# jopohl/urh

Measured on NVIDIA H100. Metric: MSamples/s IQ demod+digitize (complex64), higher is better.
Workload: dtype f32

## Files before the change

### urh_b200/csrc/dense_f32.cuh

```cuda
#pragma once
#include "dense.cuh"

struct SrcQad {
    static constexpr bool BINARY = false;
    template <typename T> __device__ __forceinline__ static int cls(T s, const UrhClassify& C, float) { return urh_classify((float)s, C); }
    template <typename T> __device__ __forceinline__ static void bits(T, const UrhClassify&, float, bool& nz, bool& ab) { nz = false; ab = false; }
    template <typename T> __device__ __forceinline__ static bool above(T, float) { return false; }
};
struct SrcQad2 {
    static constexpr bool BINARY = true;
    template <typename T> __device__ __forceinline__ static int cls(T s, const UrhClassify& C, float thr0) {
        const int c = ((float)s <= thr0) ? 0 : 1;
        return ((float)s == C.noise_value) ? -1 : c;
    }
    template <typename T> __device__ __forceinline__ static void bits(T s, const UrhClassify& C, float thr0, bool& nz, bool& ab) {
        nz = (float)s == C.noise_value;
        ab = !((float)s <= thr0) && !nz;
    }
    template <typename T> __device__ __forceinline__ static bool above(T s, float thr0) { return !((float)s <= thr0); }
};
struct SrcAbove {
    static constexpr bool BINARY = true;
    template <typename T> __device__ __forceinline__ static int cls(T s, const UrhClassify&, float thr0) { return (s > (T)thr0) ? 1 : 0; }
    template <typename T> __device__ __forceinline__ static void bits(T s, const UrhClassify&, float thr0, bool& nz, bool& ab) { nz = false; ab = s > (T)thr0; }
    template <typename T> __device__ __forceinline__ static bool above(T s, float thr0) { return s > (T)thr0; }
};
struct SrcCenter {
    static constexpr bool BINARY = true;
    template <typename T> __device__ __forceinline__ static int cls(T s, const UrhClassify&, float thr0) { return (s <= (T)thr0) ? 0 : 1; }
    template <typename T> __device__ __forceinline__ static void bits(T s, const UrhClassify&, float thr0, bool& nz, bool& ab) { nz = false; ab = !(s <= (T)thr0); }
    template <typename T> __device__ __forceinline__ static bool above(T s, float thr0) { return !(s <= (T)thr0); }
};

struct UrhSpec {
    const float* tg;
    float* margin;
    int64_t lo, hi;
    unsigned int* redone;
};

template <typename T> struct UrhVec2;
template <> struct UrhVec2<float> { typedef float2 type; };
template <> struct UrhVec2<double> { typedef double2 type; };

template <typename SRC, typename T>
__global__ void __launch_bounds__(URH_WARPS_PER_BLOCK * 32)
k_dense_f32(const T* __restrict__ x, int64_t n, int vec_in, const __grid_constant__ UrhClassify cls, int tol,
            UrhTileSummary* __restrict__ tiles, uint32_t* __restrict__ staging, int stage_cap,
            int16_t* __restrict__ init_cls, int cls_of_zero, const float* __restrict__ d_thr0 = nullptr,
            const UrhTileStats* __restrict__ tile_stats = nullptr, const UrhSpec spec = UrhSpec{}) {
    const float thr0 = d_thr0 ? *d_thr0 : cls.thr[0];
    if (d_thr0) cls_of_zero = (0.0f <= thr0) ? 0 : 1;
    const int lane = threadIdx.x & 31;
    const int64_t tile = (int64_t)blockIdx.x * URH_WARPS_PER_BLOCK + (threadIdx.x >> 5);
    const int64_t tile_start = tile * URH_TILE;
    if (tile_start >= n) return;
    const int tile_len = (int)((n - tile_start) < URH_TILE ? (n - tile_start) : URH_TILE);
    const int iters = (tile_len + 63) >> 6;
    if (tile_stats && tile_stats[tile].all_noise) {
        if (lane == 0) {
            UrhTileSummary s;
            s.first_cls = -1; s.last_cls = -1; s.head_len = tile_len; s.tail_len = tile_len; s.ncand = 0;
            tiles[tile] = s;
            if (tile_start == 0 && init_cls) *init_cls = (int16_t)-1;
        }
        return;
    }
    if (tile >= spec.lo && tile < spec.hi) {
        if (spec.margin[tile] > fabsf(__fsub_rn(thr0, *spec.tg))) return;
        if (lane == 0) atomicAdd(spec.redone, 1u);
    }
    UrhRunTracker rt;
    rt.init(tol, staging + tile * (int64_t)stage_cap);
    if (vec_in && tile_len == URH_TILE) {
        typedef typename UrhVec2<T>::type V;
        const V* p = (const V*)(x + tile_start) + lane;
        constexpr int ITERS = URH_TILE / 64;
        const bool no_noise = SRC::BINARY && tile_stats && cls.noise_value <= -4.0f && tile_stats[tile].cnt == URH_TILE;
        V cur[4], nxt[4];
#pragma unroll
        for (int j = 0; j < 4; j++) cur[j] = __ldg(p + j * 32);
        if (tile_start == 0 && lane == 0 && init_cls) *init_cls = (int16_t)(((float)cur[0].x == cls.noise_value) ? -1 : cls_of_zero);
        if (SRC::BINARY) {
            UrhTileResolve tr;
            tr.init();
#pragma unroll 1
            for (int it = 0; it < ITERS; it += 4) {
                if (it + 4 < ITERS) {
#pragma unroll
                    for (int j = 0; j < 4; j++) nxt[j] = __ldg(p + (it + 4 + j) * 32);
                }
                if (no_noise) {
#pragma unroll
                    for (int j = 0; j < 4; j++)
                        tr.keep(it + j, 0u, __ballot_sync(URH_FULL_MASK, SRC::template above<T>(cur[j].x, thr0)), 0u,
                                __ballot_sync(URH_FULL_MASK, SRC::template above<T>(cur[j].y, thr0)), lane);
                } else {
#pragma unroll
                    for (int j = 0; j < 4; j++) {
                        bool nx, ax, ny, ay;
                        SRC::template bits<T>(cur[j].x, cls, thr0, nx, ax);
                        SRC::template bits<T>(cur[j].y, cls, thr0, ny, ay);
                        tr.keep(it + j, __ballot_sync(URH_FULL_MASK, nx), __ballot_sync(URH_FULL_MASK, ax), __ballot_sync(URH_FULL_MASK, ny),
                                __ballot_sync(URH_FULL_MASK, ay), lane);
// ... 17 lines not shown
#pragma unroll
            for (int j = 0; j < 4; j++) cur[j] = nxt[j];
        }
        rt.finish(tile_len, tiles + tile, lane);
        return;
    }
    for (int it = 0; it < iters; it += 2) {
        T a0 = 0, a1 = 0, b0 = 0, b1 = 0;
        const int64_t pa = tile_start + (int64_t)it * 64 + 2 * lane;
        const int64_t pb = pa + 64;
        if (vec_in && pa + 1 < n) {
            const typename UrhVec2<T>::type v = __ldg((const typename UrhVec2<T>::type*)(x + pa));
            a0 = v.x; a1 = v.y;
        } else {
            if (pa < n) a0 = __ldg(x + pa);
            if (pa + 1 < n) a1 = __ldg(x + pa + 1);
        }
        const bool has_b = it + 1 < iters;
        if (has_b) {
            if (vec_in && pb + 1 < n) {
                const typename UrhVec2<T>::type v = __ldg((const typename UrhVec2<T>::type*)(x + pb));
                b0 = v.x; b1 = v.y;
            } else {
                if (pb < n) b0 = __ldg(x + pb);
                if (pb + 1 < n) b1 = __ldg(x + pb + 1);
            }
        }
        if (pa == 0 && init_cls) *init_cls = (int16_t)(((float)a0 == cls.noise_value) ? -1 : cls_of_zero);
        rt.feed(it, SRC::template cls<T>(a0, cls, thr0), SRC::template cls<T>(a1, cls, thr0), pa < n, pa + 1 < n, lane);
        if (has_b) rt.feed(it + 1, SRC::template cls<T>(b0, cls, thr0), SRC::template cls<T>(b1, cls, thr0), pb < n, pb + 1 < n, lane);
    }
    rt.finish(tile_len, tiles + tile, lane);
}
```

### urh_b200/csrc/digitize.cu

```cuda
#include "dense.cuh"
#include "scan.cuh"
#include "sparse.cuh"
#ifndef URH_FAST_MIN_BLOCKS
#define URH_FAST_MIN_BLOCKS 4
#endif
#include "fsk_fast.cuh"
#include "dense_f32.cuh"

#include <math.h>
#include <stdlib.h>


template <int DT, int MOD, bool DIGITIZE>
__device__ __forceinline__ void dense_iq_tile(const void* __restrict__ iq, int64_t n, const UrhDemodParams& dp, float* __restrict__ qad_out,
                                              int vec_in, int vec_out, const UrhClassify& cls, int tol, UrhTileSummary* __restrict__ tiles,
                                              uint32_t* __restrict__ staging, int stage_cap, int16_t* __restrict__ init_cls, int cls_of_zero,
                                              int64_t tile, int has_halo, UrhTileStats* __restrict__ tile_stats, const UrhFine& fine,
                                              unsigned int* s_fine, unsigned int* g_fine) {
    const int lane = threadIdx.x & 31;
    const int64_t tile_start = tile * URH_TILE;
    const int tile_len = (int)((n - tile_start) < URH_TILE ? (n - tile_start) : URH_TILE);
    const int iters = (tile_len + 63) >> 6;

    UrhRunTracker rt;
// ... 805 lines not shown
    if (urh_iq_bytes(dtype) == 0) URH_FAIL(ctx, URH_ERR_DTYPE, "Unsupported dtype");
    return URH_OK;
}

static int stream_check(urh_ctx* ctx, int64_t n, int ring, int mod_type, int dtype, bool iq) {
    if (n <= 0) URH_FAIL(ctx, URH_ERR_INVALID, "streamed call: empty capture");
    if (ring < 2 || ring > URH_STREAM_MAX_RING) URH_FAIL(ctx, URH_ERR_INVALID, "streamed call: ring of %d slots (2..%d)", ring, URH_STREAM_MAX_RING);
    if (iq && (n <= 2 || (mod_type != URH_MOD_ASK && mod_type != URH_MOD_FSK)))
        URH_FAIL(ctx, URH_ERR_INVALID, "streamed demodulation: ASK/FSK and n > 2 (PSK is a serial recurrence)");
    if (iq && urh_iq_bytes(dtype) == 0) URH_FAIL(ctx, URH_ERR_DTYPE, "Unsupported dtype");
    return URH_OK;
}

template <bool DIG>
static int stream_dense_iq(urh_ctx* ctx, int dtype, int mod_type, const char* d_src, int64_t src_slot, int64_t n, const UrhDemodParams& dp,
                           float* qad_global, const UrhClassify& cls, int tol, StreamDigitizer* dz, int64_t s0, int64_t s1, int s,
                           UrhTileStats* ts = nullptr, const UrhFine& fine = UrhFine{}) {
    const int b = urh_iq_bytes(dtype);
    const void* iq = d_src + s * src_slot + URH_STREAM_PAD - s0 * b;
    const int64_t t0 = s0 / URH_TILE, t1 = urh_div_up(s1, URH_TILE);
    UrhTileSummary* tiles = dz ? dz->tiles - t0 : nullptr;
    uint32_t* staging = dz ? dz->staging - t0 * dz->cap : nullptr;
    const int cap = dz ? dz->cap : 0;
    int16_t* init = dz ? dz->d_init : nullptr;
    const int c0 = DIG ? host_classify(0.0f, cls) : 0;
    if (mod_type == URH_MOD_ASK)
        return launch_dense_iq_m<URH_MOD_ASK, DIG>(ctx, dtype, iq, n, dp, qad_global, cls, tol, tiles, staging, cap, init, c0, 0, ts, t0, t1, fine);
    return launch_dense_iq_m<URH_MOD_FSK, DIG>(ctx, dtype, iq, n, dp, qad_global, cls, tol, tiles, staging, cap, init, c0, 0, ts, t0, t1, fine);
}

static int stream_dense_qad(urh_ctx* ctx, const float* x, int64_t s0, int64_t s1, const UrhClassify& cls, StreamDigitizer& dz,
                            const float* d_thr0 = nullptr, const UrhTileStats* ts = nullptr) {
    const int64_t nc = s1 - s0;
    const unsigned grid = (unsigned)urh_div_up(urh_div_up(nc, URH_TILE), URH_WARPS_PER_BLOCK);
    const int vec_in = (((uintptr_t)x % 8) == 0) ? 1 : 0;
    int16_t* init = s0 == 0 ? dz.d_init : nullptr;
    const int c0 = d_thr0 ? 0 : host_classify(0.0f, cls);
    const UrhTileStats* tsc = ts ? ts + s0 / URH_TILE : nullptr;
    if (cls.order == 2)
        URH_LAUNCH(ctx, (k_dense_f32<SrcQad2, float>), grid, URH_WARPS_PER_BLOCK * 32, 0, x, nc, vec_in, cls, dz.tol, dz.tiles, dz.staging,
                   dz.cap, init, c0, d_thr0, tsc);
    else
        URH_LAUNCH(ctx, (k_dense_f32<SrcQad, float>), grid, URH_WARPS_PER_BLOCK * 32, 0, x, nc, vec_in, cls, dz.tol, dz.tiles, dz.staging,
                   dz.cap, init, c0, d_thr0, tsc);
    return URH_OK;
}

struct CenterPlan;
int urh_center_chain(urh_ctx* ctx, const float* d_qad, int64_t n, const UrhTileStats* ts, int64_t max_size, int rank, int world,
                     const UrhFine* fine, CenterPlan** d_plan_out);
int urh_center_plan_result(urh_ctx* ctx, const CenterPlan* plan, const float** d_centerf, const double** d_center, const int** d_state);
int urh_center_plan_certify_stats(urh_ctx* ctx, const CenterPlan* plan, int64_t* h_dst3);

extern "C" int urh_shard_digitize(urh_ctx* ctx, const void* d_iq, int dtype, const float* d_qad_in, int64_t n, int has_halo,
                                  float noise_mag, int mod_type, float center, uint16_t tolerance, uint32_t samples_per_symbol,
                                  uint8_t bits_per_symbol, float center_spacing, float* d_qad_out, int64_t global_offset,
                                  int64_t n_total, int64_t* k) {
    if (!k) return URH_ERR_INVALID;
    *k = 0;
    ctx->pulses_k = 0;
    if (n <= 0) URH_FAIL(ctx, URH_ERR_INVALID, "empty shard");
    if (mod_type != URH_MOD_ASK && mod_type != URH_MOD_FSK) URH_FAIL(ctx, URH_ERR_INVALID, "sharded path: ASK / FSK only");
    if (!d_qad_in && urh_iq_bytes(dtype) == 0) URH_FAIL(ctx, URH_ERR_DTYPE, "Unsupported dtype");
    if (!ctx->nccl_comm) URH_FAIL(ctx, URH_ERR_INVALID, "NCCL communicator not initialised (urh_nccl_init)");
    urh_arena_reset(ctx);
    UrhClassify cls;
    URH_CHECK(fill_classify(ctx, &cls, mod_type, center, bits_per_symbol, center_spacing));
    const int tol = tolerance;
    const int64_t ntiles = urh_div_up(n, URH_TILE);
    const int cap = stage_cap_for(tol);
    UrhTileSummary* tiles;
    uint32_t* staging;
    int16_t* d_init;
    URH_CHECK(urh_arena(ctx, (size_t)ntiles, &tiles));
    URH_CHECK(urh_arena(ctx, (size_t)ntiles * cap, &staging));
    URH_CHECK(urh_arena(ctx, 8, &d_init));
    URH_CUDA(ctx, cudaMemsetAsync(d_init, 0, 16, ctx->stream));
// ... 117 lines not shown
                                                             ts, t0, t1, fine, speculate ? &spec : nullptr)));
    }
    CenterPlan* plan = nullptr;
    URH_CHECK(urh_center_chain(ctx, d_qad_out, n, ts, max_size, sharded ? ctx->nccl_rank : 0, sharded ? ctx->nccl_world : 1,
                               fine.gh ? &fine : nullptr, &plan));
    const float* d_centerf;
    const double* d_center;
    const int* d_state;
    urh_center_plan_result(ctx, plan, &d_centerf, &d_center, &d_state);
    int64_t rows = 0;
    if (sc) {
        URH_CUDA(ctx, cudaMemcpyAsync(ctx->h_mail + 40, d_center, sizeof(double), cudaMemcpyDeviceToHost, ctx->stream));
        URH_CUDA(ctx, cudaMemcpyAsync(ctx->h_mail + 41, d_state, sizeof(int), cudaMemcpyDeviceToHost, ctx->stream));
        URH_CHECK(urh_center_plan_certify_stats(ctx, plan, ctx->h_mail + 42));
        URH_CUDA(ctx, cudaMemcpyAsync(ctx->h_mail + 45, (const int64_t*)ctx->center_prefix + ntiles, sizeof(int64_t), cudaMemcpyDeviceToHost,
                                      ctx->stream));
        URH_CUDA(ctx, cudaStreamSynchronize(ctx->stream));
        int st0 = 0;
        memcpy(&st0, ctx->h_mail + 41, sizeof(int));
        if (st0 == 1) {
            StreamDigitizer dz;
            URH_CHECK(dz.init(ctx, n, scs, tol, mod_type == URH_MOD_ASK, samples_per_symbol));
            for (int64_t s0 = 0; s0 < n; s0 += scs) {
                const int64_t s1 = s0 + scs < n ? s0 + scs : n;
                URH_CHECK(stream_dense_qad(ctx, d_qad_out + s0, s0, s1, cls, dz, d_centerf, ts));
                URH_CHECK(dz.finish(ctx, s0, s1));
            }
            rows = dz.rows;
        }
        *sc->kept = ctx->h_mail[45];
    } else {
        URH_CUDA(ctx, cudaMemsetAsync(d_init, 0, 16, ctx->stream));
        const int vec_in = (((uintptr_t)d_qad_out % 8) == 0) ? 1 : 0;
        URH_LAUNCH(ctx, (k_dense_f32<SrcQad2, float>), (unsigned)urh_div_up(ntiles, URH_WARPS_PER_BLOCK), URH_WARPS_PER_BLOCK * 32, 0,
                   (const float*)d_qad_out, n, vec_in, cls, tol, tiles, staging, cap, d_init, 0, d_centerf, (const UrhTileStats*)ts, spec);
        URH_CUDA(ctx, cudaMemcpyAsync(ctx->h_mail + 40, d_center, sizeof(double), cudaMemcpyDeviceToHost, ctx->stream));
        URH_CUDA(ctx, cudaMemcpyAsync(ctx->h_mail + 41, d_state, sizeof(int), cudaMemcpyDeviceToHost, ctx->stream));
        URH_CHECK(urh_center_plan_certify_stats(ctx, plan, ctx->h_mail + 42));
        ctx->h_mail[46] = 0;
        if (speculate) URH_CUDA(ctx, cudaMemcpyAsync(ctx->h_mail + 46, spec.redone, sizeof(unsigned int), cudaMemcpyDeviceToHost, ctx->stream));
        if (sharded)
            URH_CHECK(urh_finish_shard(ctx, n, tol, mod_type == URH_MOD_ASK, samples_per_symbol, tiles, staging, cap, d_init, global_offset, n_total, &rows));
        else
            URH_CHECK(urh_finish_local(ctx, n, tol, mod_type == URH_MOD_ASK, samples_per_symbol, tiles, staging, cap, d_init, &rows));
    }
    memcpy(center, ctx->h_mail + 40, sizeof(double));
    int st = 0;
    memcpy(&st, ctx->h_mail + 41, sizeof(int));
    *center_state = st;
    ctx->center_cert[0] = ctx->h_mail[42];
    ctx->center_cert[1] = fine.gh ? URH_FINE_NB : 0;
    ctx->center_cert[2] = ctx->h_mail[44];
    const int64_t redone = (spec.hi > spec.lo) ? ctx->h_mail[46] : 0;
    ctx->spec_stats[0] = spec.hi - spec.lo;
    ctx->spec_stats[1] = spec.hi - spec.lo - redone;
    ctx->spec_stats[2] = redone;
    if (st != 1) {
        ctx->pulses_k = 0;
        rows = 0;
    }
    *k = rows;
    return URH_OK;
}

extern "C" int urh_speculate_stats(urh_ctx* ctx, int64_t* h_out3) {
    for (int i = 0; i < 3; i++) h_out3[i] = ctx->spec_stats[i];
    return URH_OK;
}
// ... 325 lines not shown
```

### urh_b200/csrc/finish.cu

```cuda
#include "sparse.cuh"
#include "tilescan.cuh"

#include <limits.h>

#define CLS_NONE INT_MIN

struct __align__(16) CandAgg {
    int64_t cnt;
    int32_t last_cls;
    int32_t pad;
};
struct CandOp {
    __device__ __forceinline__ CandAgg operator()(const CandAgg& a, const CandAgg& b) const {
        CandAgg r;
        r.cnt = a.cnt + b.cnt;
        r.last_cls = (b.last_cls != CLS_NONE) ? b.last_cls : a.last_cls;
        r.pad = 0;
        return r;
    }
};
struct __align__(16) FireAgg {
    int64_t fired;
    int64_t last_pos;
};
struct FireOp {
    __device__ __forceinline__ FireAgg operator()(const FireAgg& a, const FireAgg& b) const {
        FireAgg r;
        r.fired = a.fired + b.fired;
        r.last_pos = (b.last_pos >= 0) ? b.last_pos : a.last_pos;
        return r;
    }
};

struct ScanRunCarry {
    const UrhTileSummary* tiles;
    int64_t n;
    RunCarry* carry;
    __device__ __forceinline__ RunCarry load(int64_t t) const {
        const int64_t rem = n - t * URH_TILE;
        const int tile_len = rem < URH_TILE ? (int)rem : URH_TILE;
        const UrhTileSummary s = tiles[t];
        RunCarry r;
        r.len = s.tail_len;
        r.cls = s.last_cls;
        r.flags = (s.head_len == tile_len) ? 1 : 0;
        return r;
    }
    __device__ __forceinline__ void post(int64_t t, const RunCarry& excl, const RunCarry&) const { carry[t] = excl; }
};

struct ScanCandidates {
    const UrhTileSummary* tiles;
    const uint32_t* staging;
    int stage_cap;
    const RunCarry* carry;
    const RunCarry* xcarry;
    int tol;
    int32_t* head_rel;
    int32_t* prev_cls;
    __device__ __forceinline__ CandAgg load(int64_t t) const {
        const UrhTileSummary s = tiles[t];
        RunCarry c = carry[t];
        if (xcarry) c = RunCarryOp()(*xcarry, c);
        int64_t start_len = 0;
        if (!(c.flags & 2) && c.cls == s.first_cls) start_len = c.len;
        int32_t rel = -1;
        if (start_len <= tol && (int64_t)tol < start_len + s.head_len) rel = (int32_t)(tol - start_len);
        head_rel[t] = rel;
        CandAgg r;
        r.cnt = (int64_t)s.ncand + (rel >= 0 ? 1 : 0);
        r.last_cls = CLS_NONE;
        if (s.ncand > 0) r.last_cls = (int32_t)(staging[t * (int64_t)stage_cap + s.ncand - 1] & 0xffffu) - 1;
        else if (rel >= 0) r.last_cls = s.first_cls;
        r.pad = 0;
        return r;
    }
    __device__ __forceinline__ void post(int64_t t, const CandAgg& excl, const CandAgg&) const { prev_cls[t] = excl.last_cls; }
};

struct ScanFirings {
    const UrhTileSummary* tiles;
    const uint32_t* staging;
    int stage_cap;
    const int32_t* head_rel;
    const int32_t* prev_cls;
    const int16_t* d_prev0;
    int64_t global_offset;
    int64_t* row_off;
    int64_t* prev_fired;
    __device__ __forceinline__ FireAgg load(int64_t t) const {
        const UrhTileSummary s = tiles[t];
        int prev = prev_cls[t];
        if (prev == CLS_NONE) prev = *d_prev0;
        const int64_t base = t * URH_TILE + global_offset;
        FireAgg r;
        r.fired = 0;
        r.last_pos = -1;
        const int32_t rel = head_rel[t];
        if (rel >= 0) {
            const int c = s.first_cls;
            if (c != prev) { r.fired++; r.last_pos = base + rel; }
            prev = c;
        }
        const uint32_t* st = staging + t * (int64_t)stage_cap;
        for (int j = 0; j < s.ncand; j++) {
            const uint32_t v = st[j];
            const int c = (int)(v & 0xffffu) - 1;
            if (c != prev) { r.fired++; r.last_pos = base + (v >> 16); }
            prev = c;
        }
        return r;
    }
    __device__ __forceinline__ void post(int64_t t, const FireAgg& excl, const FireAgg&) const {
        row_off[t] = excl.fired;
        prev_fired[t] = excl.last_pos;
    }
};

__global__ void __launch_bounds__(256) k_finish_rows(const UrhTileSummary* __restrict__ tiles, const uint32_t* __restrict__ staging,
                                                    int stage_cap, const int32_t* __restrict__ head_rel, const int32_t* __restrict__ prev_cls,
                                                    const int16_t* __restrict__ d_prev0, const int64_t* __restrict__ row_off,
                                                    const int64_t* __restrict__ prev_fired, const int64_t* __restrict__ d_xprev_fired,
                                                    int64_t ntiles, int64_t global_offset, int64_t n_total, int tol, int is_ask, int64_t sps,
                                                    int emit_tail, int64_t row_base, int64_t* __restrict__ out, int64_t cap_rows,
                                                    int64_t* __restrict__ d_out) {
    const int64_t t = (int64_t)blockIdx.x * blockDim.x + threadIdx.x;
    if (t >= ntiles) return;
    const UrhTileSummary s = tiles[t];
    int prev = prev_cls[t];
    if (prev == CLS_NONE) prev = *d_prev0;
    int64_t pp = prev_fired[t];
    if (pp < 0) pp = *d_xprev_fired;
    int64_t idx = row_off[t];
    const int64_t base = t * URH_TILE + global_offset;
    auto fire = [&](int64_t p, int c) {
        if (c != prev) {
            const int64_t rec = (pp >= 0) ? (p - pp) : (p + 1 - tol);
            int64_t st = prev;
            if (is_ask && st == -1 && rec < sps) st = 0;
            if (idx < cap_rows) *((longlong2*)out + idx) = make_longlong2(st, rec);
            idx++;
            pp = p;
        }
        prev = c;
    };
    const int32_t rel = head_rel[t];
    if (rel >= 0) fire(base + rel, s.first_cls);
    const uint32_t* st = staging + t * (int64_t)stage_cap;
    for (int j = 0; j < s.ncand; j++) {
        const uint32_t v = st[j];
        fire(base + (v >> 16), (int)(v & 0xffffu) - 1);
    }
    if (t == ntiles - 1) {
        const int64_t fired = idx;
        if (emit_tail && (is_ask || row_base + fired < n_total)) {
            if (idx < cap_rows) *((longlong2*)out + idx) = make_longlong2(prev, (pp >= 0) ? (n_total - 1 - pp) : (n_total - tol));
            idx++;
        }
        d_out[0] = idx;
        d_out[1] = fired;
    }
}

struct ScanMergeRows {
    const int64_t* raw;
    int64_t rows;
    int64_t n_total;
    int has_tail;
    int64_t* out;
    int64_t* d_k;
    const int64_t* prev_last;
    int64_t row_base;
    __device__ __forceinline__ int64_t load(int64_t r) const {
        if (r == 0) return (prev_last && raw[0] == *prev_last) ? 0 : 1;
        return raw[2 * r] != raw[2 * r - 2] ? 1 : 0;
    }
    __device__ __forceinline__ void post(int64_t r, const int64_t& excl, const int64_t& head) const {
        const bool is_tail = has_tail && r == rows - 1;
        if (is_tail && row_base + excl >= n_total) {
            *d_k = excl;
            return;
        }
        const int64_t o = excl + head - 1;
        if (head) out[2 * o] = raw[2 * r];
        atomicAdd((unsigned long long*)&out[2 * o + 1], (unsigned long long)raw[2 * r + 1]);
        if (r == rows - 1) *d_k = o + 1;
    }
};
struct AddI64 {
    __device__ __forceinline__ int64_t operator()(int64_t a, int64_t b) const { return a + b; }
};

__global__ void k_pack_stage1(const int16_t* __restrict__ d_init, const RunCarry* __restrict__ total, int64_t* __restrict__ msg) {
// ... 35 lines not shown
__global__ void k_chain_start(const int16_t* __restrict__ d_init, UrhChain* __restrict__ chain) {
    chain->run.len = 0; chain->run.cls = 0; chain->run.flags = 2 | 1;
    chain->prev_fired = -1;
    chain->last_state = INT64_MIN;
    chain->prev_cls = *d_init;
}
__global__ void k_chain_advance(UrhChain* __restrict__ chain, const RunCarry* __restrict__ tot_run, const CandAgg* __restrict__ tot_cand,
                                const FireAgg* __restrict__ tot_fire) {
    chain->run = RunCarryOp()(chain->run, *tot_run);
    if (tot_cand->last_cls != CLS_NONE) chain->prev_cls = (int16_t)tot_cand->last_cls;
    if (tot_fire->last_pos >= 0) chain->prev_fired = tot_fire->last_pos;
}
__global__ void k_chain_last_row(UrhChain* __restrict__ chain, const int64_t* __restrict__ table, int64_t rows) {
    if (rows > 0) chain->last_state = table[2 * (rows - 1)];
}

int urh_coll_allgather(urh_ctx* ctx, const void* d_send, void* d_recv, size_t bytes_per_rank);
extern "C" int urh_p2p_check(urh_ctx* ctx);

struct FinishShard {
    int rank, world;
    int64_t global_offset;
    int64_t n_total;
    int emit_tail;
    UrhChain* chain;
    int64_t row_base, rows_cap;
};

static int finish_tiles(urh_ctx* ctx, int64_t n, int tol, bool is_ask, uint32_t sps, const UrhTileSummary* tiles, const uint32_t* staging,
                        int stage_cap, const int16_t* d_init, const FinishShard& sh, int64_t* k) {
    const int64_t ntiles = urh_div_up(n, URH_TILE);
    const bool sharded = sh.world > 1;
    UrhChain* chain = sh.chain;
    RunCarry* carry;
    int32_t *head_rel, *prev_cls;
    int64_t *row_off, *prev_fired, *d_small;
    URH_CHECK(urh_arena(ctx, (size_t)ntiles, &carry));
    URH_CHECK(urh_arena(ctx, (size_t)ntiles, &head_rel));
    URH_CHECK(urh_arena(ctx, (size_t)ntiles, &prev_cls));
    URH_CHECK(urh_arena(ctx, (size_t)ntiles, &row_off));
    URH_CHECK(urh_arena(ctx, (size_t)ntiles, &prev_fired));
    URH_CHECK(urh_arena(ctx, (size_t)(32 + 8 * (sharded ? sh.world : 0)), &d_small));
    URH_CUDA(ctx, cudaMemsetAsync(d_small, 0xff, 4 * sizeof(int64_t), ctx->stream));
    RunCarry* d_tot_run = (RunCarry*)(d_small + 4);
    CandAgg* d_tot_cand = (CandAgg*)(d_small + 6);
    FireAgg* d_tot_fire = (FireAgg*)(d_small + 8);
    RunCarry* d_xcarry = (RunCarry*)(d_small + 10);
    int16_t* d_prev0 = (int16_t*)(d_small + 12);
    int64_t* d_xprev = d_small + 13;
    int64_t* d_msg1 = d_small + 16;
    int64_t* d_all1 = d_small + 32;
    int64_t* d_all2 = d_all1 + 4 * (sharded ? sh.world : 0);
    int64_t* d_all3 = d_all2 + 2 * (sharded ? sh.world : 0);

    if (chain && sh.global_offset == 0) URH_LAUNCH(ctx, k_chain_start, 1, 1, 0, d_init, chain);
    RunCarry rc_ident;
    rc_ident.len = 0; rc_ident.cls = 0; rc_ident.flags = 2 | 1;
    ScanRunCarry fa;
    fa.tiles = tiles; fa.n = n; fa.carry = carry;
    URH_CHECK((urhts::scan<RunCarry, RunCarryOp, ScanRunCarry>(ctx, ntiles, rc_ident, RunCarryOp(), fa, d_tot_run)));
    if (sharded) {
        URH_LAUNCH(ctx, k_pack_stage1, 1, 1, 0, d_init, (const RunCarry*)d_tot_run, d_msg1);
        URH_TL_MARK(ctx, "x4 run carry: enter");
        URH_CHECK(urh_coll_allgather(ctx, d_msg1, d_all1, 4 * sizeof(int64_t)));
        URH_TL_MARK(ctx, "x4 run carry: done");
        URH_LAUNCH(ctx, k_fold_carry, 1, 1, 0, (const int64_t*)d_all1, sh.rank, d_xcarry);
    }
    ScanCandidates fb;
    fb.tiles = tiles; fb.staging = staging; fb.stage_cap = stage_cap; fb.carry = carry;
    fb.xcarry = sharded ? d_xcarry : (chain ? &chain->run : nullptr);
    fb.tol = tol; fb.head_rel = head_rel; fb.prev_cls = prev_cls;
    CandAgg ca_ident;
    ca_ident.cnt = 0; ca_ident.last_cls = CLS_NONE; ca_ident.pad = 0;
    URH_CHECK((urhts::scan<CandAgg, CandOp, ScanCandidates>(ctx, ntiles, ca_ident, CandOp(), fb, d_tot_cand)));
    const int16_t* prev0 = chain ? &chain->prev_cls : d_init;
    if (sharded) {
        URH_TL_MARK(ctx, "x5 candidates: enter");
        URH_CHECK(urh_coll_allgather(ctx, d_tot_cand, d_all2, sizeof(CandAgg)));
        URH_TL_MARK(ctx, "x5 candidates: done");
        URH_LAUNCH(ctx, k_fold_prev_cls, 1, 1, 0, (const int64_t*)d_all2, sh.rank, (const int64_t*)d_all1, d_prev0);
        prev0 = d_prev0;
    }
    ScanFirings fc;
    fc.tiles = tiles; fc.staging = staging; fc.stage_cap = stage_cap; fc.head_rel = head_rel; fc.prev_cls = prev_cls; fc.d_prev0 = prev0;
    fc.global_offset = sh.global_offset; fc.row_off = row_off; fc.prev_fired = prev_fired;
    FireAgg fi_ident;
    fi_ident.fired = 0; fi_ident.last_pos = -1;
    URH_CHECK((urhts::scan<FireAgg, FireOp, ScanFirings, 4>(ctx, ntiles, fi_ident, FireOp(), fc, d_tot_fire)));
    const int64_t* xprev = chain ? &chain->prev_fired : d_small + 2;
    if (sharded) {
        URH_TL_MARK(ctx, "x6 firings: enter");
        URH_CHECK(urh_coll_allgather(ctx, d_tot_fire, d_all3, sizeof(FireAgg)));
        URH_TL_MARK(ctx, "x6 firings: done");
        URH_LAUNCH(ctx, k_fold_prev_fired, 1, 1, 0, (const int64_t*)d_all3, sh.rank, d_xprev);
        xprev = d_xprev;
    }

    int64_t cap_rows = (int64_t)ctx->pulses_cap_rows;
    const int64_t guess = n / 64 + 1024;
    if (!chain && cap_rows < guess) {
        URH_CHECK(urh_ensure_pulses(ctx, (size_t)guess));
        cap_rows = (int64_t)ctx->pulses_cap_rows;
    }
    const int64_t row_base = chain ? sh.row_base : 0;
    int64_t* raw = ctx->pulses + 2 * row_base;
    int64_t raw_cap = chain ? sh.rows_cap : cap_rows;
    if (is_ask) URH_CHECK(urh_arena(ctx, (size_t)raw_cap * 2, &raw));
    int64_t got[2] = {0, 0};
    for (int attempt = 0; attempt < 2; attempt++) {
        URH_LAUNCH(ctx, k_finish_rows, (unsigned)urh_div_up(ntiles, 256), 256, 0, tiles, staging, stage_cap, (const int32_t*)head_rel,
                   (const int32_t*)prev_cls, prev0, (const int64_t*)row_off, (const int64_t*)prev_fired, xprev, ntiles, sh.global_offset,
                   sh.n_total, tol, is_ask ? 1 : 0, (int64_t)sps, sh.emit_tail, row_base, raw, raw_cap, d_small);
        if (sharded && attempt == 0) URH_TL_MARK(ctx, "rows written");
        URH_CHECK(urh_read_i64(ctx, d_small, 2, got));
        if (sharded) URH_CHECK(urh_p2p_check(ctx));
        if (got[0] <= raw_cap) break;
        if (attempt == 1 || chain) URH_FAIL(ctx, URH_ERR_CUDA, "finish_tiles: row buffer overflow after regrowth");
        if (is_ask) {
            URH_CHECK(urh_arena(ctx, (size_t)got[0] * 2, &raw));
            raw_cap = got[0];
        } else {
            URH_CHECK(urh_ensure_pulses(ctx, (size_t)got[0]));
            raw = ctx->pulses;
            raw_cap = (int64_t)ctx->pulses_cap_rows;
        }
    }
    if (chain) URH_LAUNCH(ctx, k_chain_advance, 1, 1, 0, chain, (const RunCarry*)d_tot_run, (const CandAgg*)d_tot_cand, (const FireAgg*)d_tot_fire);
    int64_t K = got[0];
    if (is_ask && K > 0) {
        if (!chain) URH_CHECK(urh_ensure_pulses(ctx, (size_t)K));
        int64_t* out = ctx->pulses + 2 * row_base;
        URH_CUDA(ctx, cudaMemsetAsync(out, 0, (size_t)K * 2 * sizeof(int64_t), ctx->stream));
        ScanMergeRows fm;
        fm.raw = raw; fm.rows = K; fm.n_total = sh.n_total; fm.has_tail = (sh.emit_tail && K > got[1]) ? 1 : 0; fm.out = out;
        fm.d_k = d_small;
        fm.prev_last = (chain && row_base > 0) ? &chain->last_state : nullptr;
        fm.row_base = row_base;
        URH_CHECK((urhts::scan<int64_t, AddI64, ScanMergeRows>(ctx, K, (int64_t)0, AddI64(), fm, (int64_t*)nullptr)));
        URH_CHECK(urh_read_i64(ctx, d_small, 1, &K));
        if (chain) URH_LAUNCH(ctx, k_chain_last_row, 1, 1, 0, chain, (const int64_t*)ctx->pulses, row_base + K);
    }
    ctx->pulses_k = row_base + K;
    *k = K;
// ... 30 lines not shown
```

Measured before the change: 206,600.

## Warp-cooperative candidate walks and sparse dense-tile scheduling in finish pipeline

Adds a pre-pass kernel that summarises each tile's staged candidates (first, last class, inner firing count, last firing position) using warp-cooperative loads and ballots. The candidate and firing scans then read this compact summary instead of looping serially over staging per thread. The row-emission kernel now uses one warp per tile with shuffle-based prefix scans instead of one thread per tile. The dense classify kernel is split into a plain variant and a sparse variant that does noise and speculation checks lane-parallel and only runs the warps with tiles left to do. This adds an extra kernel launch and more code complexity in exchange for less warp divergence and fewer serial global loads.

Result: faster. 212,100, median of 6 (+2.7%).

```diff
diff --git a/urh_b200/csrc/dense_f32.cuh b/urh_b200/csrc/dense_f32.cuh
--- a/urh_b200/csrc/dense_f32.cuh
+++ b/urh_b200/csrc/dense_f32.cuh
@@ -44,32 +44,13 @@
 template <> struct UrhVec2<double> { typedef double2 type; };
 
 template <typename SRC, typename T>
-__global__ void __launch_bounds__(URH_WARPS_PER_BLOCK * 32)
-k_dense_f32(const T* __restrict__ x, int64_t n, int vec_in, const __grid_constant__ UrhClassify cls, int tol,
-            UrhTileSummary* __restrict__ tiles, uint32_t* __restrict__ staging, int stage_cap,
-            int16_t* __restrict__ init_cls, int cls_of_zero, const float* __restrict__ d_thr0 = nullptr,
-            const UrhTileStats* __restrict__ tile_stats = nullptr, const UrhSpec spec = UrhSpec{}) {
-    const float thr0 = d_thr0 ? *d_thr0 : cls.thr[0];
-    if (d_thr0) cls_of_zero = (0.0f <= thr0) ? 0 : 1;
-    const int lane = threadIdx.x & 31;
-    const int64_t tile = (int64_t)blockIdx.x * URH_WARPS_PER_BLOCK + (threadIdx.x >> 5);
+__device__ __forceinline__ void dense_f32_tile(const T* __restrict__ x, int64_t n, int vec_in, const UrhClassify& cls, int tol,
+                                               UrhTileSummary* __restrict__ tiles, uint32_t* __restrict__ staging, int stage_cap,
+                                               int16_t* __restrict__ init_cls, int cls_of_zero, float thr0,
+                                               const UrhTileStats* __restrict__ tile_stats, int64_t tile, int lane) {
     const int64_t tile_start = tile * URH_TILE;
-    if (tile_start >= n) return;
     const int tile_len = (int)((n - tile_start) < URH_TILE ? (n - tile_start) : URH_TILE);
     const int iters = (tile_len + 63) >> 6;
-    if (tile_stats && tile_stats[tile].all_noise) {
-        if (lane == 0) {
-            UrhTileSummary s;
-            s.first_cls = -1; s.last_cls = -1; s.head_len = tile_len; s.tail_len = tile_len; s.ncand = 0;
-            tiles[tile] = s;
-            if (tile_start == 0 && init_cls) *init_cls = (int16_t)-1;
-        }
-        return;
-    }
-    if (tile >= spec.lo && tile < spec.hi) {
-        if (spec.margin[tile] > fabsf(__fsub_rn(thr0, *spec.tg))) return;
-        if (lane == 0) atomicAdd(spec.redone, 1u);
-    }
     UrhRunTracker rt;
     rt.init(tol, staging + tile * (int64_t)stage_cap);
     if (vec_in && tile_len == URH_TILE) {
@@ -153,3 +134,76 @@
     }
     rt.finish(tile_len, tiles + tile, lane);
 }
+
+__device__ __forceinline__ void dense_noise_tile(int64_t n, UrhTileSummary* __restrict__ tiles, int16_t* __restrict__ init_cls, int64_t tile) {
+    const int64_t tile_start = tile * URH_TILE;
+    const int tile_len = (int)((n - tile_start) < URH_TILE ? (n - tile_start) : URH_TILE);
+    UrhTileSummary s;
+    s.first_cls = -1; s.last_cls = -1; s.head_len = tile_len; s.tail_len = tile_len; s.ncand = 0;
+    tiles[tile] = s;
+    if (tile_start == 0 && init_cls) *init_cls = (int16_t)-1;
+}
+
+template <typename SRC, typename T>
+__global__ void __launch_bounds__(URH_WARPS_PER_BLOCK * 32)
+k_dense_f32(const T* __restrict__ x, int64_t n, int vec_in, const __grid_constant__ UrhClassify cls, int tol,
+            UrhTileSummary* __restrict__ tiles, uint32_t* __restrict__ staging, int stage_cap,
+            int16_t* __restrict__ init_cls, int cls_of_zero, const float* __restrict__ d_thr0 = nullptr) {
+    const float thr0 = d_thr0 ? *d_thr0 : cls.thr[0];
+    if (d_thr0) cls_of_zero = (0.0f <= thr0) ? 0 : 1;
+    const int64_t tile = (int64_t)blockIdx.x * URH_WARPS_PER_BLOCK + (threadIdx.x >> 5);
+    if (tile * URH_TILE >= n) return;
+    dense_f32_tile<SRC, T>(x, n, vec_in, cls, tol, tiles, staging, stage_cap, init_cls, cls_of_zero, thr0, nullptr, tile, threadIdx.x & 31);
+}
+
+template <typename SRC, typename T>
+__global__ void __launch_bounds__(URH_WARPS_PER_BLOCK * 32)
+k_dense_f32_sparse(const T* __restrict__ x, int64_t n, int vec_in, const __grid_constant__ UrhClassify cls, int tol,
+                   UrhTileSummary* __restrict__ tiles, uint32_t* __restrict__ staging, int stage_cap,
+                   int16_t* __restrict__ init_cls, int cls_of_zero, const float* __restrict__ d_thr0,
+                   const UrhTileStats* __restrict__ tile_stats, const UrhSpec spec) {
+    const float thr0 = d_thr0 ? *d_thr0 : cls.thr[0];
+    if (d_thr0) cls_of_zero = (0.0f <= thr0) ? 0 : 1;
+    const int lane = threadIdx.x & 31;
+    const int64_t ntiles = (n + URH_TILE - 1) / URH_TILE;
+    const int64_t nwarps = (int64_t)gridDim.x * URH_WARPS_PER_BLOCK;
+    const float gap = spec.lo < spec.hi ? fabsf(__fsub_rn(thr0, *spec.tg)) : 0.0f;
+    for (int64_t g = ((int64_t)blockIdx.x * URH_WARPS_PER_BLOCK + (threadIdx.x >> 5)) * 32; g < ntiles; g += nwarps * 32) {
+        const int64_t tile = g + lane;
+        bool todo = false, redo = false;
+        if (tile < ntiles) {
+            if (tile_stats && tile_stats[tile].all_noise) {
+                dense_noise_tile(n, tiles, init_cls, tile);
+            } else if (tile >= spec.lo && tile < spec.hi) {
+                redo = !(spec.margin[tile] > gap);
+                todo = redo;
+            } else {
+                todo = true;
+            }
+        }
+        unsigned m = __ballot_sync(URH_FULL_MASK, todo);
+        const unsigned r = __ballot_sync(URH_FULL_MASK, redo);
+        if (r && lane == 0) atomicAdd(spec.redone, (unsigned)__popc(r));
+        while (m) {
+            const int k = __ffs(m) - 1;
+            m &= m - 1;
+            dense_f32_tile<SRC, T>(x, n, vec_in, cls, tol, tiles, staging, stage_cap, init_cls, cls_of_zero, thr0, tile_stats, g + k, lane);
+        }
+    }
+}
+
+template <typename SRC, typename T>
+static inline int launch_dense_qad(urh_ctx* ctx, const T* x, int64_t n, int vec_in, const UrhClassify& cls, int tol, UrhTileSummary* tiles,
+                                    uint32_t* staging, int stage_cap, int16_t* init_cls, int cls_of_zero, const float* d_thr0 = nullptr,
+                                    const UrhTileStats* tile_stats = nullptr, const UrhSpec& spec = UrhSpec{}) {
+    const int64_t ntiles = urh_div_up(n, URH_TILE);
+    if (!tile_stats && spec.lo >= spec.hi) {
+        URH_LAUNCH(ctx, (k_dense_f32<SRC, T>), (unsigned)urh_div_up(ntiles, URH_WARPS_PER_BLOCK), URH_WARPS_PER_BLOCK * 32, 0, x, n, vec_in,
+                   cls, tol, tiles, staging, stage_cap, init_cls, cls_of_zero, d_thr0);
+        return URH_OK;
+    }
+    const int64_t want = urh_div_up(ntiles, 32 * URH_WARPS_PER_BLOCK), most = (int64_t)ctx->sm_count * 8;
+    URH_LAUNCH(ctx, (k_dense_f32_sparse<SRC, T>), (unsigned)(want < most ? want : most), URH_WARPS_PER_BLOCK * 32, 0, x, n, vec_in, cls, tol,
+               tiles, staging, stage_cap, init_cls, cls_of_zero, d_thr0, tile_stats, spec);
+    return URH_OK;
+}
diff --git a/urh_b200/csrc/digitize.cu b/urh_b200/csrc/digitize.cu
--- a/urh_b200/csrc/digitize.cu
+++ b/urh_b200/csrc/digitize.cu
@@ -861,17 +861,14 @@
 static int stream_dense_qad(urh_ctx* ctx, const float* x, int64_t s0, int64_t s1, const UrhClassify& cls, StreamDigitizer& dz,
                             const float* d_thr0 = nullptr, const UrhTileStats* ts = nullptr) {
     const int64_t nc = s1 - s0;
-    const unsigned grid = (unsigned)urh_div_up(urh_div_up(nc, URH_TILE), URH_WARPS_PER_BLOCK);
     const int vec_in = (((uintptr_t)x % 8) == 0) ? 1 : 0;
     int16_t* init = s0 == 0 ? dz.d_init : nullptr;
     const int c0 = d_thr0 ? 0 : host_classify(0.0f, cls);
     const UrhTileStats* tsc = ts ? ts + s0 / URH_TILE : nullptr;
     if (cls.order == 2)
-        URH_LAUNCH(ctx, (k_dense_f32<SrcQad2, float>), grid, URH_WARPS_PER_BLOCK * 32, 0, x, nc, vec_in, cls, dz.tol, dz.tiles, dz.staging,
-                   dz.cap, init, c0, d_thr0, tsc);
+        URH_CHECK((launch_dense_qad<SrcQad2, float>(ctx, x, nc, vec_in, cls, dz.tol, dz.tiles, dz.staging, dz.cap, init, c0, d_thr0, tsc)));
     else
-        URH_LAUNCH(ctx, (k_dense_f32<SrcQad, float>), grid, URH_WARPS_PER_BLOCK * 32, 0, x, nc, vec_in, cls, dz.tol, dz.tiles, dz.staging,
-                   dz.cap, init, c0, d_thr0, tsc);
+        URH_CHECK((launch_dense_qad<SrcQad, float>(ctx, x, nc, vec_in, cls, dz.tol, dz.tiles, dz.staging, dz.cap, init, c0, d_thr0, tsc)));
     return URH_OK;
 }
 
@@ -1055,8 +1052,8 @@
     } else {
         URH_CUDA(ctx, cudaMemsetAsync(d_init, 0, 16, ctx->stream));
         const int vec_in = (((uintptr_t)d_qad_out % 8) == 0) ? 1 : 0;
-        URH_LAUNCH(ctx, (k_dense_f32<SrcQad2, float>), (unsigned)urh_div_up(ntiles, URH_WARPS_PER_BLOCK), URH_WARPS_PER_BLOCK * 32, 0,
-                   (const float*)d_qad_out, n, vec_in, cls, tol, tiles, staging, cap, d_init, 0, d_centerf, (const UrhTileStats*)ts, spec);
+        URH_CHECK((launch_dense_qad<SrcQad2, float>(ctx, (const float*)d_qad_out, n, vec_in, cls, tol, tiles, staging, cap, d_init, 0, d_centerf,
+                                                    (const UrhTileStats*)ts, spec)));
         URH_CUDA(ctx, cudaMemcpyAsync(ctx->h_mail + 40, d_center, sizeof(double), cudaMemcpyDeviceToHost, ctx->stream));
         URH_CUDA(ctx, cudaMemcpyAsync(ctx->h_mail + 41, d_state, sizeof(int), cudaMemcpyDeviceToHost, ctx->stream));
         URH_CHECK(urh_center_plan_certify_stats(ctx, plan, ctx->h_mail + 42));
diff --git a/urh_b200/csrc/finish.cu b/urh_b200/csrc/finish.cu
--- a/urh_b200/csrc/finish.cu
+++ b/urh_b200/csrc/finish.cu
@@ -31,6 +31,99 @@
         return r;
     }
 };
+
+struct __align__(16) TileCands {
+    int32_t ncand;
+    uint32_t first;
+    int16_t last_cls;
+    int16_t inner;
+    int16_t inner_last;
+    int16_t head_cls;
+};
+
+__device__ __forceinline__ int cand_cls(uint32_t v) { return (int)(v & 0xffffu) - 1; }
+
+__device__ __forceinline__ int tile_firings(const TileCands& tc, int32_t rel, int prev, int* last_rel, int* cls_after) {
+    int fired = 0, last = -1;
+    if (rel >= 0) {
+        if (tc.head_cls != prev) { fired++; last = rel; }
+        prev = tc.head_cls;
+    }
+    if (tc.ncand > 0) {
+        if (cand_cls(tc.first) != prev) { fired++; last = (int)(tc.first >> 16); }
+        fired += tc.inner;
+        if (tc.inner_last >= 0) last = tc.inner_last;
+        prev = tc.last_cls;
+    }
+    *last_rel = last;
+    *cls_after = prev;
+    return fired;
+}
+
+#define WALK_BATCH 8
+static unsigned tile_walk_grid(const urh_ctx* ctx, int64_t ntiles) {
+    const int64_t want = urh_div_up(ntiles, 32 * 8), most = (int64_t)ctx->sm_count * 8;
+    return (unsigned)(want < 1 ? 1 : (want < most ? want : most));
+}
+
+__global__ void __launch_bounds__(256) k_tile_cands(const UrhTileSummary* __restrict__ tiles, const uint32_t* __restrict__ staging,
+                                                   int stage_cap, int64_t ntiles, TileCands* __restrict__ out) {
+    const int lane = threadIdx.x & 31;
+    const int64_t nwarps = (int64_t)gridDim.x * (blockDim.x >> 5);
+    for (int64_t g = ((int64_t)blockIdx.x * (blockDim.x >> 5) + (threadIdx.x >> 5)) * 32; g < ntiles; g += nwarps * 32) {
+        const int here = ntiles - g < 32 ? (int)(ntiles - g) : 32;
+        int my_nc = 0, my_head = 0;
+        if (lane < here) {
+            const UrhTileSummary s = tiles[g + lane];
+            my_nc = s.ncand;
+            my_head = s.first_cls;
+        }
+        TileCands mine;
+        auto walk = [&](int i, uint32_t v0) -> TileCands {
+            const int nc = __shfl_sync(URH_FULL_MASK, my_nc, i);
+            const uint32_t* st = staging + (g + i) * (int64_t)stage_cap;
+            int prevc = 0, inner = 0, inner_last = -1;
+            const uint32_t first = __shfl_sync(URH_FULL_MASK, v0, 0);
+            for (int j0 = 0; j0 < nc; j0 += 32) {
+                const int j = j0 + lane;
+                const uint32_t v = j0 == 0 ? v0 : ((j < nc) ? __ldg(st + j) : 0u);
+                const int c = cand_cls(v);
+                int pc = __shfl_up_sync(URH_FULL_MASK, c, 1);
+                if (lane == 0) pc = prevc;
+                const unsigned m = __ballot_sync(URH_FULL_MASK, j > 0 && j < nc && c != pc);
+                inner += __popc(m);
+                const uint32_t vl = __shfl_sync(URH_FULL_MASK, v, m ? 31 - __clz(m) : 0);
+                if (m) inner_last = (int)(vl >> 16);
+                prevc = __shfl_sync(URH_FULL_MASK, c, min(31, nc - 1 - j0));
+            }
+            TileCands r;
+            r.ncand = nc;
+            r.first = nc > 0 ? first : 0u;
+            r.last_cls = (int16_t)prevc;
+            r.inner = (int16_t)inner;
+            r.inner_last = (int16_t)inner_last;
+            r.head_cls = (int16_t)__shfl_sync(URH_FULL_MASK, my_head, i);
+            return r;
+        };
+        for (int b = 0; b < here; b += WALK_BATCH) {
+            uint32_t w[WALK_BATCH];
+#pragma unroll
+            for (int u = 0; u < WALK_BATCH; u++) {
+                const int i = b + u;
+                const int nc = __shfl_sync(URH_FULL_MASK, my_nc, i & 31);
+                w[u] = (i < here && lane < nc) ? __ldg(staging + (g + i) * (int64_t)stage_cap + lane) : 0u;
+            }
+#pragma unroll
+            for (int u = 0; u < WALK_BATCH; u++) {
+                if (b + u < here) {
+                    const TileCands r = walk(b + u, w[u]);
+                    if (lane == b + u) mine = r;
+                }
+            }
+        }
+        if (lane < here) out[g + lane] = mine;
+    }
+}
 
 struct ScanRunCarry {
     const UrhTileSummary* tiles;
@@ -51,8 +144,7 @@
 
 struct ScanCandidates {
     const UrhTileSummary* tiles;
-    const uint32_t* staging;
-    int stage_cap;
+    const TileCands* cands;
     const RunCarry* carry;
     const RunCarry* xcarry;
     int tol;
@@ -70,7 +162,7 @@
         CandAgg r;
         r.cnt = (int64_t)s.ncand + (rel >= 0 ? 1 : 0);
         r.last_cls = CLS_NONE;
-        if (s.ncand > 0) r.last_cls = (int32_t)(staging[t * (int64_t)stage_cap + s.ncand - 1] & 0xffffu) - 1;
+        if (s.ncand > 0) r.last_cls = cands[t].last_cls;
         else if (rel >= 0) r.last_cls = s.first_cls;
         r.pad = 0;
         return r;
@@ -79,9 +171,7 @@
 };
 
 struct ScanFirings {
-    const UrhTileSummary* tiles;
-    const uint32_t* staging;
-    int stage_cap;
+    const TileCands* cands;
     const int32_t* head_rel;
     const int32_t* prev_cls;
     const int16_t* d_prev0;
@@ -89,26 +179,12 @@
     int64_t* row_off;
     int64_t* prev_fired;
     __device__ __forceinline__ FireAgg load(int64_t t) const {
-        const UrhTileSummary s = tiles[t];
         int prev = prev_cls[t];
         if (prev == CLS_NONE) prev = *d_prev0;
-        const int64_t base = t * URH_TILE + global_offset;
+        int last_rel, cls_after;
         FireAgg r;
-        r.fired = 0;
-        r.last_pos = -1;
-        const int32_t rel = head_rel[t];
-        if (rel >= 0) {
-            const int c = s.first_cls;
-            if (c != prev) { r.fired++; r.last_pos = base + rel; }
-            prev = c;
-        }
-        const uint32_t* st = staging + t * (int64_t)stage_cap;
-        for (int j = 0; j < s.ncand; j++) {
-            const uint32_t v = st[j];
-            const int c = (int)(v & 0xffffu) - 1;
-            if (c != prev) { r.fired++; r.last_pos = base + (v >> 16); }
-            prev = c;
-        }
+        r.fired = tile_firings(cands[t], head_rel[t], prev, &last_rel, &cls_after);
+        r.last_pos = last_rel >= 0 ? t * URH_TILE + global_offset + last_rel : -1;
         return r;
     }
     __device__ __forceinline__ void post(int64_t t, const FireAgg& excl, const FireAgg&) const {
@@ -117,48 +193,109 @@
     }
 };
 
-__global__ void __launch_bounds__(256) k_finish_rows(const UrhTileSummary* __restrict__ tiles, const uint32_t* __restrict__ staging,
+__global__ void __launch_bounds__(256) k_finish_rows(const TileCands* __restrict__ cands, const uint32_t* __restrict__ staging,
                                                     int stage_cap, const int32_t* __restrict__ head_rel, const int32_t* __restrict__ prev_cls,
                                                     const int16_t* __restrict__ d_prev0, const int64_t* __restrict__ row_off,
                                                     const int64_t* __restrict__ prev_fired, const int64_t* __restrict__ d_xprev_fired,
                                                     int64_t ntiles, int64_t global_offset, int64_t n_total, int tol, int is_ask, int64_t sps,
                                                     int emit_tail, int64_t row_base, int64_t* __restrict__ out, int64_t cap_rows,
                                                     int64_t* __restrict__ d_out) {
-    const int64_t t = (int64_t)blockIdx.x * blockDim.x + threadIdx.x;
-    if (t >= ntiles) return;
-    const UrhTileSummary s = tiles[t];
-    int prev = prev_cls[t];
-    if (prev == CLS_NONE) prev = *d_prev0;
-    int64_t pp = prev_fired[t];
-    if (pp < 0) pp = *d_xprev_fired;
-    int64_t idx = row_off[t];
-    const int64_t base = t * URH_TILE + global_offset;
-    auto fire = [&](int64_t p, int c) {
-        if (c != prev) {
-            const int64_t rec = (pp >= 0) ? (p - pp) : (p + 1 - tol);
-            int64_t st = prev;
-            if (is_ask && st == -1 && rec < sps) st = 0;
-            if (idx < cap_rows) *((longlong2*)out + idx) = make_longlong2(st, rec);
-            idx++;
-            pp = p;
+    const int lane = threadIdx.x & 31;
+    const unsigned below = (1u << lane) - 1u;
+    const int prev0 = *d_prev0;
+    const int64_t xprev = *d_xprev_fired;
+    const int64_t nwarps = (int64_t)gridDim.x * (blockDim.x >> 5);
+    for (int64_t g = ((int64_t)blockIdx.x * (blockDim.x >> 5) + (threadIdx.x >> 5)) * 32; g < ntiles; g += nwarps * 32) {
+        const int here = ntiles - g < 32 ? (int)(ntiles - g) : 32;
+        TileCands my_tc;
+        int32_t my_rel = -1, my_prev = 0;
+        int64_t my_row = 0, my_pp = -1;
+        my_tc.ncand = 0;
+        if (lane < here) {
+            my_tc = cands[g + lane];
+            my_rel = head_rel[g + lane];
+            my_prev = prev_cls[g + lane];
+            my_row = row_off[g + lane];
+            my_pp = prev_fired[g + lane];
         }
-        prev = c;
-    };
-    const int32_t rel = head_rel[t];
-    if (rel >= 0) fire(base + rel, s.first_cls);
-    const uint32_t* st = staging + t * (int64_t)stage_cap;
-    for (int j = 0; j < s.ncand; j++) {
-        const uint32_t v = st[j];
-        fire(base + (v >> 16), (int)(v & 0xffffu) - 1);
-    }
-    if (t == ntiles - 1) {
-        const int64_t fired = idx;
-        if (emit_tail && (is_ask || row_base + fired < n_total)) {
-            if (idx < cap_rows) *((longlong2*)out + idx) = make_longlong2(prev, (pp >= 0) ? (n_total - 1 - pp) : (n_total - tol));
-            idx++;
+        if (my_prev == CLS_NONE) my_prev = prev0;
+        if (my_pp < 0) my_pp = xprev;
+        int last_rel = -1, cls_after = 0;
+        const int my_fired = lane < here ? tile_firings(my_tc, my_rel, my_prev, &last_rel, &cls_after) : 0;
+        auto walk = [&](int i, uint32_t v0) {
+            const int64_t t = g + i;
+            const int fired = __shfl_sync(URH_FULL_MASK, my_fired, i);
+            int prev = __shfl_sync(URH_FULL_MASK, my_prev, i);
+            int64_t pp = __shfl_sync(URH_FULL_MASK, my_pp, i);
+            int64_t idx = __shfl_sync(URH_FULL_MASK, my_row, i);
+            if (fired > 0) {
+                const int32_t rel = __shfl_sync(URH_FULL_MASK, my_rel, i);
+                const int nc = __shfl_sync(URH_FULL_MASK, my_tc.ncand, i);
+                const int head_cls = __shfl_sync(URH_FULL_MASK, (int)my_tc.head_cls, i);
+                const int h = rel >= 0 ? 1 : 0;
+                const int m = nc + h;
+                const int64_t base = t * URH_TILE + global_offset;
+                const uint32_t* st = staging + t * (int64_t)stage_cap;
+                for (int e0 = 0; e0 < m; e0 += 32) {
+                    const int e = e0 + lane, j = e - h;
+                    const uint32_t v = e0 == 0 ? v0 : ((j < nc) ? __ldg(st + j) : 0u);
+                    const bool is_head = h && e == 0;
+                    const int c = is_head ? head_cls : cand_cls(v);
+                    const int p = is_head ? rel : (int)(v >> 16);
+                    int pc = __shfl_up_sync(URH_FULL_MASK, c, 1);
+                    if (lane == 0) pc = prev;
+                    const bool fire = e < m && c != pc;
+                    const unsigned mask = __ballot_sync(URH_FULL_MASK, fire);
+                    int incl = fire ? p : -1;
+#pragma unroll
+                    for (int off = 1; off < 32; off <<= 1) {
+                        const int o = __shfl_up_sync(URH_FULL_MASK, incl, off);
+                        if (lane >= off) incl = max(incl, o);
+                    }
+                    int excl = __shfl_up_sync(URH_FULL_MASK, incl, 1);
+                    if (lane == 0) excl = -1;
+                    if (fire) {
+                        const int64_t pos = base + p;
+                        const int64_t pf = excl >= 0 ? base + excl : pp;
+                        const int64_t rec = (pf >= 0) ? (pos - pf) : (pos + 1 - tol);
+                        int64_t sv = pc;
+                        if (is_ask && sv == -1 && rec < sps) sv = 0;
+                        const int64_t r = idx + __popc(mask & below);
+                        if (r < cap_rows) *((longlong2*)out + r) = make_longlong2(sv, rec);
+                    }
+                    idx += __popc(mask);
+                    const int last = __shfl_sync(URH_FULL_MASK, incl, 31);
+                    if (last >= 0) pp = base + last;
+                    prev = __shfl_sync(URH_FULL_MASK, c, min(31, m - 1 - e0));
+                }
+            } else {
+                prev = __shfl_sync(URH_FULL_MASK, cls_after, i);
+            }
+            if (t == ntiles - 1 && lane == 0) {
+                const int64_t fired_all = idx;
+                if (emit_tail && (is_ask || row_base + fired_all < n_total)) {
+                    if (idx < cap_rows) *((longlong2*)out + idx) = make_longlong2(prev, (pp >= 0) ? (n_total - 1 - pp) : (n_total - tol));
+                    idx++;
+                }
+                d_out[0] = idx;
+                d_out[1] = fired_all;
+            }
+        };
+        for (int b = 0; b < here; b += WALK_BATCH) {
+            uint32_t w[WALK_BATCH];
+#pragma unroll
+            for (int u = 0; u < WALK_BATCH; u++) {
+                const int i = b + u;
+                const int h = __shfl_sync(URH_FULL_MASK, my_rel, i & 31) >= 0 ? 1 : 0;
+                const int nc = __shfl_sync(URH_FULL_MASK, my_tc.ncand, i & 31);
+                const int fired = __shfl_sync(URH_FULL_MASK, my_fired, i & 31);
+                const int j = lane - h;
+                w[u] = (i < here && fired > 0 && j >= 0 && j < nc) ? __ldg(staging + (g + i) * (int64_t)stage_cap + j) : 0u;
+            }
+#pragma unroll
+            for (int u = 0; u < WALK_BATCH; u++)
+                if (b + u < here) walk(b + u, w[u]);
         }
-        d_out[0] = idx;
-        d_out[1] = fired;
     }
 }
 
@@ -260,9 +397,11 @@
     const int64_t ntiles = urh_div_up(n, URH_TILE);
     const bool sharded = sh.world > 1;
     UrhChain* chain = sh.chain;
+    TileCands* cands;
     RunCarry* carry;
     int32_t *head_rel, *prev_cls;
     int64_t *row_off, *prev_fired, *d_small;
+    URH_CHECK(urh_arena(ctx, (size_t)ntiles, &cands));
     URH_CHECK(urh_arena(ctx, (size_t)ntiles, &carry));
     URH_CHECK(urh_arena(ctx, (size_t)ntiles, &head_rel));
     URH_CHECK(urh_arena(ctx, (size_t)ntiles, &prev_cls));
@@ -282,6 +421,8 @@
     int64_t* d_all3 = d_all2 + 2 * (sharded ? sh.world : 0);
 
     if (chain && sh.global_offset == 0) URH_LAUNCH(ctx, k_chain_start, 1, 1, 0, d_init, chain);
+    const unsigned walk_grid = tile_walk_grid(ctx, ntiles);
+    URH_LAUNCH(ctx, k_tile_cands, walk_grid, 256, 0, tiles, staging, stage_cap, ntiles, cands);
     RunCarry rc_ident;
     rc_ident.len = 0; rc_ident.cls = 0; rc_ident.flags = 2 | 1;
     ScanRunCarry fa;
@@ -295,7 +436,7 @@
         URH_LAUNCH(ctx, k_fold_carry, 1, 1, 0, (const int64_t*)d_all1, sh.rank, d_xcarry);
     }
     ScanCandidates fb;
-    fb.tiles = tiles; fb.staging = staging; fb.stage_cap = stage_cap; fb.carry = carry;
+    fb.tiles = tiles; fb.cands = cands; fb.carry = carry;
     fb.xcarry = sharded ? d_xcarry : (chain ? &chain->run : nullptr);
     fb.tol = tol; fb.head_rel = head_rel; fb.prev_cls = prev_cls;
     CandAgg ca_ident;
@@ -310,11 +451,11 @@
         prev0 = d_prev0;
     }
     ScanFirings fc;
-    fc.tiles = tiles; fc.staging = staging; fc.stage_cap = stage_cap; fc.head_rel = head_rel; fc.prev_cls = prev_cls; fc.d_prev0 = prev0;
+    fc.cands = cands; fc.head_rel = head_rel; fc.prev_cls = prev_cls; fc.d_prev0 = prev0;
     fc.global_offset = sh.global_offset; fc.row_off = row_off; fc.prev_fired = prev_fired;
     FireAgg fi_ident;
     fi_ident.fired = 0; fi_ident.last_pos = -1;
-    URH_CHECK((urhts::scan<FireAgg, FireOp, ScanFirings, 4>(ctx, ntiles, fi_ident, FireOp(), fc, d_tot_fire)));
+    URH_CHECK((urhts::scan<FireAgg, FireOp, ScanFirings>(ctx, ntiles, fi_ident, FireOp(), fc, d_tot_fire)));
     const int64_t* xprev = chain ? &chain->prev_fired : d_small + 2;
     if (sharded) {
         URH_TL_MARK(ctx, "x6 firings: enter");
@@ -336,7 +477,7 @@
     if (is_ask) URH_CHECK(urh_arena(ctx, (size_t)raw_cap * 2, &raw));
     int64_t got[2] = {0, 0};
     for (int attempt = 0; attempt < 2; attempt++) {
-        URH_LAUNCH(ctx, k_finish_rows, (unsigned)urh_div_up(ntiles, 256), 256, 0, tiles, staging, stage_cap, (const int32_t*)head_rel,
+        URH_LAUNCH(ctx, k_finish_rows, walk_grid, 256, 0, (const TileCands*)cands, staging, stage_cap, (const int32_t*)head_rel,
                    (const int32_t*)prev_cls, prev0, (const int64_t*)row_off, (const int64_t*)prev_fired, xprev, ntiles, sh.global_offset,
                    sh.n_total, tol, is_ask ? 1 : 0, (int64_t)sps, sh.emit_tail, row_base, raw, raw_cap, d_small);
         if (sharded && attempt == 0) URH_TL_MARK(ctx, "rows written");
```
